# ingonyama-zk/blaze

Measured on AMD Instinct MI355X. Metric: BLS12-381 MSM/s at 2^26, higher is better.
Workload: dtype u32 registers holding 28-bit limbs (381-bit Fq, Montgomery)

## Files before the change

### blaze_amd/csrc/arena.hip

```cpp
#include "msm_engine.hpp"

#include <atomic>
#include <cstdlib>
#include <string>

namespace blz {

static std::mutex g_arena_mu;
static std::map<int, Arena*> g_arenas;

Arena& arena_for(int device_id) {
    std::lock_guard<std::mutex> lk(g_arena_mu);
    auto it = g_arenas.find(device_id);
    if (it == g_arenas.end()) it = g_arenas.emplace(device_id, new Arena()).first;
    return *it->second;
}

ArenaExtent* arena_find(Arena& a, uint64_t pos, size_t len) {
    if (pos + len < pos) return nullptr;
    for (auto& e : a.ext)
        if (pos >= e.start && pos + len <= e.start + e.len) return &e;
    return nullptr;
}

uint32_t* arena_flag_acquire(Arena& a) {
    if (!a.build_flags) {
        if (hipMalloc((void**)&a.build_flags, 256 * sizeof(uint32_t)) != hipSuccess) {
            (void)hipGetLastError();
            a.build_flags = nullptr;
            return nullptr;
        }
        a.flag_free.clear();
        for (int i = 255; i >= 0; --i) a.flag_free.push_back((uint16_t)i);
    }
    if (a.flag_free.empty()) return nullptr;
    uint32_t* f = a.build_flags + a.flag_free.back();
    a.flag_free.pop_back();
    return f;
}
void arena_flag_release(Arena& a, uint32_t*& f) {
    if (f && a.build_flags && f >= a.build_flags && f < a.build_flags + 256) a.flag_free.push_back((uint16_t)(f - a.build_flags));
    f = nullptr;
}

void arena_drop_build(Arena& a, ArenaExtent& x) {
    if (x.build.tab) (void)hipFree(x.build.tab);
    if (x.build.done) (void)hipEventDestroy(x.build.done);
    if (x.build.t0) (void)hipEventDestroy(x.build.t0);
    arena_flag_release(a, x.build.flag);
    x.build = ArenaExtent::TableBuild();
}
void arena_drop_table(Arena& a, ArenaExtent& x) {
    for (auto& t : x.tables)
        if (t.p) (void)hipFree(t.p);
    x.tables.clear();
    x.tab_dirty_lo = x.tab_dirty_hi = 0;
    arena_drop_build(a, x);
}

void arena_free_extent(Arena& a, ArenaExtent& x) {
    if (x.raw) {
        if (x.imported) (void)hipIpcCloseMemHandle(x.raw);
        else (void)hipFree(x.raw);
    }
    if (x.mont) (void)hipFree(x.mont);
    arena_drop_table(a, x);
    if (x.shadow_ready) (void)hipEventDestroy(x.shadow_ready);
    if (x.diet_ev) (void)hipEventDestroy(x.diet_ev);
    arena_flag_release(a, x.diet_flag);
    x = ArenaExtent();
}

uint64_t arena_next_epoch() {
    static std::atomic<uint64_t> next{1};
    return next.fetch_add(1);
}

static size_t format_point_bytes(int format_id) { return (format_id & 0xff) == BLZ_BN254 ? 64 : 96; }

int arena_restore_raw(Arena& a, ArenaExtent& e, hipStream_t st) {
    (void)a;
    if (e.diet == 1) e.diet = 0;
    if (e.diet != 2) return BLZ_OK;
    const size_t ps = format_point_bytes(e.mont_curve), mp = mont_point_bytes(e.mont_curve & 0xff);
    void* raw = nullptr;
    BLZ_HIP(hipMalloc(&raw, e.cap), BLZ_ERR_UNKNOWN);
    int rc = msm_points_from_mont(e.mont_curve, e.mont, raw, e.len / ps, st);
    if (rc == BLZ_OK) rc = sync_stream_bounded(st, "arena: raw bytes back from the Montgomery copy");
    if (rc != BLZ_OK) {
        if (!wait_timed_out()) (void)hipFree(raw);
// ... 280 lines not shown
```

### blaze_amd/csrc/arena_tables.hip

```cpp
#include <chrono>
#include <thread>

#include "msm_handle.hpp"

namespace blz {

bool wants_table_mode(const blz_msm* h) { return h->pf == 1 && h->window_table != 0; }

int arena_points_mont(blz_msm* h, uint64_t pos, uint32_t npts, const void** out, bool even) {
    *out = nullptr;
    const size_t ps = point_size(h), mp = mont_point_bytes(h->curve);
    const size_t len = (size_t)npts * ps;
    Arena& A = arena_for(h->device);
    std::lock_guard<std::mutex> lk(A.mu);
    ArenaExtent* e = arena_find(A, pos, len);
    if (!e)
        return fail(BLZ_ERR_INVALID_PARAM, "HBM bases: no loaded extent covers [%llu, +%zu) on device %d",
                    (unsigned long long)pos, len, h->device);
    const uint32_t phase = (uint32_t)((pos - e->start) % ps);
    const size_t cap_pts = (e->cap - phase) / ps, ext_pts = (e->len - phase) / ps;
    const uint64_t first = (pos - e->start - phase) / ps;
    if (even) {
        const ArenaExtent::PrecompCheck& C = e->pcheck;
        if ((first & 7u) || C.state != 1 || C.curve != h->curve || C.phase != phase || first < C.first || first + npts > C.first + C.npts) return BLZ_OK;
    }
    const int fmt = h->eng.format_id() | (even ? 1 << 16 : 0);
    const size_t want_bytes = (even ? (cap_pts / 8) * 4 : cap_pts) * mp;
    if (e->mont_curve != fmt || e->mont_phase != phase || e->mont_bytes < want_bytes) {
        BLZ_TRY(arena_restore_raw(A, *e, h->eng.stream));
        if (e->mont) {
            BLZ_TRY(sync_device_bounded("replacing a Montgomery shadow"));
            (void)hipFree(e->mont);
            e->mont = nullptr;
        }
        e->mont_bytes = want_bytes + 16;
        BLZ_HIP(hipMalloc(&e->mont, e->mont_bytes), BLZ_ERR_UNKNOWN);
        e->mont_curve = fmt;
        e->mont_phase = phase;
        e->dirty_lo = 0;
        e->dirty_hi = e->len;
        e->shadow_recorded = false;
    }
    if (!e->shadow_ready) BLZ_HIP(hipEventCreateWithFlags(&e->shadow_ready, hipEventDisableTiming), BLZ_ERR_UNKNOWN);
    if (e->shadow_recorded) BLZ_HIP(hipStreamWaitEvent(h->eng.stream, e->shadow_ready, 0), BLZ_ERR_UNKNOWN);
    if (e->dirty_lo < e->dirty_hi) {
        uint64_t lo = e->dirty_lo > phase ? (e->dirty_lo - phase) / ps : 0;
        uint64_t hi = e->dirty_hi > phase ? (e->dirty_hi - phase + ps - 1) / ps : 0;
        if (hi > ext_pts) hi = ext_pts;
        if (even) {
            const uint64_t elo = lo / 8, ehi = hi / 8 < ext_pts / 8 ? (hi + 7) / 8 : ext_pts / 8;
            if (elo < ehi)
                BLZ_TRY(h->eng.points_to_mont_even((const char*)e->raw + phase + elo * 8 * ps, (char*)e->mont + elo * 4 * mp, (uint32_t)((ehi - elo) * 4)));
        } else if (lo < hi) {
            BLZ_TRY(h->eng.points_to_mont((const char*)e->raw + phase + lo * ps, (char*)e->mont + lo * mp, (uint32_t)(hi - lo)));
        }
        BLZ_HIP(hipEventRecord(e->shadow_ready, h->eng.stream), BLZ_ERR_UNKNOWN);
        e->shadow_recorded = true;
        e->dirty_lo = e->dirty_hi = 0;
    }
    *out = (const char*)e->mont + (even ? first / 8 * 4 : first) * mp;
    if (even) h->pc_info[3] = e->mont_bytes;
    else if (!wants_table_mode(h)) BLZ_TRY(arena_diet_step(A, *e, ps, h->eng.stream));
    return BLZ_OK;
}

int arena_precompute_check(blz_msm* h, uint64_t pos, uint32_t nelem, bool* ok, uint64_t* checked_elems) {
    *ok = false;
    if (checked_elems) *checked_elems = nelem;
    const size_t ps = point_size(h);
// ... 76 lines not shown
    std::lock_guard<std::mutex> lk(A.mu);
    if (kernel_done) arena_flag_release(A, flag);
    BLZ_TRY(rc);
    ArenaExtent* e = arena_find(A, pos, len);
    if (!e || e->epoch != epoch) {
        BLZ_LOG(1, "precompute plan: the extent was written while its table was being checked: exact path for this task");
        return BLZ_OK;
    }
    ArenaExtent::PrecompCheck& C = e->pcheck;
    if (C.gen != gen) {
        BLZ_LOG(1, "precompute plan: another check of the extent committed while this one ran: exact path for this task");
        return BLZ_OK;
    }
    ++C.gen;
    C.state = flag_h ? 2 : 1;
    C.curve = h->curve;
    C.phase = phase;
    if (!partial) {
        C.first = first;
        C.npts = (uint64_t)nelem * 8;
    }
    C.redo_lo = C.redo_hi = 0;
    C.ms = ms;
    *ok = flag_h == 0;
    if (checked_elems) *checked_elems = C.npts / 8;
    h->pc_info[1] = (uint64_t)C.state;
    h->pc_info[2] = (uint64_t)(ms * 1000.0f);
    BLZ_LOG(1, "precompute plan: %s%llu elements checked: the table %s (%.1f ms)", partial ? "rewritten span, " : "", (unsigned long long)chk_elems,
            flag_h ? "is NOT B_j = 2^32 B_(j-1) over on-curve bases: exact path (8n points, 32-bit chunks)" : "is consistent: 4n even bases, 64-bit chunks", ms);
    return BLZ_OK;
}

constexpr uint32_t TABLE_BUILD_CHUNK = 3u << 16;
int arena_points_table(blz_msm* h, uint64_t pos, uint32_t npts, const void** out, int* c_out, int chunk_budget) {
    *out = nullptr;
    *c_out = 0;
    const size_t ps = point_size(h), mp = mont_point_bytes(h->curve);
    const size_t len = (size_t)npts * ps;
    Arena& A = arena_for(h->device);
    std::lock_guard<std::mutex> lk(A.mu);
    ArenaExtent* e = arena_find(A, pos, len);
    if (!e)
        return fail(BLZ_ERR_INVALID_PARAM, "HBM bases: no loaded extent covers [%llu, +%zu) on device %d",
                    (unsigned long long)pos, len, h->device);
    if (npts == 0) return BLZ_OK;
    BLZ_TRY(arena_restore_raw(A, *e, h->eng.stream));
    const uint32_t phase = (uint32_t)((pos - e->start) % ps);
    const uint64_t first = (pos - e->start - phase) / ps;
    const int fmt = h->eng.format_id();
    const int lo = h->range_hi ? h->range_lo : 0, hi = h->range_hi ? h->range_hi : 256;
    const int need = hi - lo < 256 ? hi - lo + 1 : 257;
    const int want_c = table_window_bits(npts, need);
    if (want_c == 0) return BLZ_OK;
    ArenaExtent::TableBuild& B = e->build;
    auto enqueue_chunks = [&](int budget) -> int {
        hipStream_t st = h->eng.stream;
        const uint64_t nchunks = (B.npts + TABLE_BUILD_CHUNK - 1) / TABLE_BUILD_CHUNK;
        if (B.next_chunk >= nchunks || budget == 0) return BLZ_OK;
        if (!A.scratch_event) BLZ_HIP(hipEventCreateWithFlags(&A.scratch_event, hipEventDisableTiming), BLZ_ERR_UNKNOWN);
        if (A.scratch_recorded) BLZ_HIP(hipStreamWaitEvent(st, A.scratch_event, 0), BLZ_ERR_UNKNOWN);
        for (; B.next_chunk < nchunks && budget != 0; ++B.next_chunk, --budget) {
            const uint64_t p0 = B.next_chunk * TABLE_BUILD_CHUNK;
            const uint32_t cnt = (uint32_t)(B.npts - p0 < TABLE_BUILD_CHUNK ? B.npts - p0 : TABLE_BUILD_CHUNK);
            if (B.next_chunk == 0) BLZ_HIP(hipEventRecord(B.t0, st), BLZ_ERR_UNKNOWN);
            BLZ_TRY(h->eng.build_table((const char*)e->raw + B.phase + (B.first + p0) * ps, (char*)B.tab + p0 * (size_t)B.W * mp, cnt, B.c, B.W, B.lo,
                                       A.build_scratch, B.flag, st));
        }
        BLZ_HIP(hipEventRecord(B.done, st), BLZ_ERR_UNKNOWN);
        B.recorded = true;
        BLZ_HIP(hipEventRecord(A.scratch_event, st), BLZ_ERR_UNKNOWN);
        A.scratch_recorded = true;
        return BLZ_OK;
    };
    hipError_t bq = hipErrorNotReady;
    if (B.tab) {
        const uint64_t nchunks = (B.npts + TABLE_BUILD_CHUNK - 1) / TABLE_BUILD_CHUNK;
        if (B.next_chunk >= nchunks && B.recorded) {
            bq = hipEventQuery(B.done);
            if (bq != hipSuccess && bq != hipErrorNotReady) { (void)hipGetLastError(); return fail(BLZ_ERR_UNKNOWN, "window table build failed: %s", hipGetErrorString(bq)); }
        }
    }
    if (B.tab && bq == hipSuccess) {
        uint32_t flag_h = 0;
        float ms = 0;
        BLZ_HIP(hipMemcpy(&flag_h, B.flag, 4, hipMemcpyDeviceToHost), BLZ_ERR_READ);
        (void)hipEventElapsedTime(&ms, B.t0, B.done);
        if (flag_h) {
            BLZ_LOG(1, "window table: a base has a multiple at infinity (a point of even order): plain path for this extent");
            BLZ_TRY(sync_device_bounded("dropping a refused window table"));
            (void)hipFree(B.tab);
            (void)hipEventDestroy(B.done);
            (void)hipEventDestroy(B.t0);
            arena_flag_release(A, B.flag);
            B = ArenaExtent::TableBuild();
            e->table_refused = true;
            return BLZ_OK;
        }
        ArenaExtent::WindowTable t;
        t.p = B.tab;
        t.bytes = B.bytes;
        t.format = B.format;
        t.phase = B.phase;
        t.first = B.first;
        t.npts = B.npts;
        t.c = B.c;
        t.W = B.W;
        t.lo = B.lo;
        t.hi = B.hi;
        t.build_ms = ms;
        e->tables.push_back(t);
        B.tab = nullptr;
        (void)hipEventDestroy(B.done);
        (void)hipEventDestroy(B.t0);
        arena_flag_release(A, B.flag);
        B = ArenaExtent::TableBuild();
        BLZ_LOG(1, "window table: %llu bases x %d windows of %d bits, %.1f MiB, complete %.1f ms after its first chunk", (unsigned long long)t.npts,
                t.W, t.c, t.bytes / 1048576.0, ms);
    }
    if (e->tab_dirty_lo < e->tab_dirty_hi && !e->tables.empty()) {
        BLZ_TRY(sync_device_bounded("window table: drain before the rewritten bases are re-tabulated"));
        uint32_t* pflag = arena_flag_acquire(A);
        if (pflag && hipMemsetAsync(pflag, 0, 4, h->eng.stream) != hipSuccess) {
            (void)hipGetLastError();
            arena_flag_release(A, pflag);
        }
        bool patched = false;
        for (size_t k = e->tables.size(); k-- > 0;) {
            ArenaExtent::WindowTable& t = e->tables[k];
            const uint64_t plo = e->tab_dirty_lo > t.phase ? (e->tab_dirty_lo - t.phase) / ps : 0;
            const uint64_t phi = e->tab_dirty_hi > t.phase ? (e->tab_dirty_hi - t.phase + ps - 1) / ps : 0;
            const uint64_t lo_p = plo > t.first ? plo : t.first, hi_p = phi < t.first + t.npts ? phi : t.first + t.npts;
            if (lo_p >= hi_p) continue;
            if (t.format != fmt || !pflag || A.build_scratch_bytes < h->eng.table_scratch_bytes(t.W) + 16) {
                (void)hipFree(t.p);
                e->tables.erase(e->tables.begin() + (long)k);
                continue;
            }
            BLZ_TRY(h->eng.build_table((const char*)e->raw + t.phase + lo_p * ps, (char*)t.p + (lo_p - t.first) * (size_t)t.W * mp, (uint32_t)(hi_p - lo_p), t.c,
                                       t.W, t.lo, A.build_scratch, pflag, h->eng.stream));
            patched = true;
        }
        if (!patched) arena_flag_release(A, pflag);
        if (patched) {
            uint32_t flag_h = 0;
            BLZ_WAIT(h, sync_stream_bounded(h->eng.stream, "window table: rewritten bases re-tabulated"));
            const hipError_t he_flag = hipMemcpy(&flag_h, pflag, 4, hipMemcpyDeviceToHost);
            arena_flag_release(A, pflag);
            BLZ_HIP(he_flag, BLZ_ERR_READ);
            if (flag_h) {
                BLZ_LOG(1, "window table: a rewritten base has a multiple at infinity (a point of even order): plain path for this extent");
                arena_drop_table(A, *e);
                e->table_refused = true;
                return BLZ_OK;
            }
            BLZ_LOG(1, "window table: rows of the rewritten bases re-tabulated (bytes [%llu, %llu) of the extent)", (unsigned long long)e->tab_dirty_lo,
                    (unsigned long long)e->tab_dirty_hi);
        }
        e->tab_dirty_lo = e->tab_dirty_hi = 0;
    }
    const ArenaExtent::WindowTable* T = nullptr;
    for (const auto& t : e->tables)
        if (t.format == fmt && t.phase == phase && first >= t.first && first + npts <= t.first + t.npts && t.lo == lo && t.hi == hi) T = &t;
    if (T && T->c != want_c) return BLZ_OK;
    if (!T) {
        if (B.tab) {
            if (B.format == fmt && B.phase == phase && first >= B.first && first + npts <= B.first + B.npts && B.lo == lo && B.hi == hi)
                BLZ_TRY(enqueue_chunks(chunk_budget));
            return BLZ_OK;
        }
        if (e->table_refused) return BLZ_OK;
        if (e->tables.size() >= ArenaExtent::MAX_TABLES) {
            BLZ_LOG(1, "window table: the extent already holds %zu tables: plain path for this handle", e->tables.size());
            return BLZ_OK;
        }
        const int c = want_c, W = table_windows(c, need);
        const size_t bytes = (size_t)npts * W * mp + 16;
        size_t free_b = 0, total_b = 0;
        BLZ_HIP(hipMemGetInfo(&free_b, &total_b), BLZ_ERR_UNKNOWN);
        const size_t scratch_b = h->eng.table_scratch_bytes(W) + 16;
        const size_t workspace = (size_t)npts * W * 32 + ((size_t)1 << (c - 1)) * 256 + ((size_t)1 << 30);
        if (free_b < bytes + scratch_b + workspace) {
            BLZ_LOG(1, "window table: %zu bytes for %u bases (c = %d, %d windows) do not fit beside the workspace (%zu free): plain path",
                    bytes, npts, c, W, free_b);
            e->table_refused = true;
            return BLZ_OK;
        }
        if (A.build_scratch_bytes < scratch_b) {
            if (A.build_scratch) {
                BLZ_TRY(sync_device_bounded("growing the window-table scratch"));
                (void)hipFree(A.build_scratch);
                A.build_scratch = nullptr;
                A.build_scratch_bytes = 0;
            }
            if (hipMalloc(&A.build_scratch, scratch_b) != hipSuccess) {
                (void)hipGetLastError();
                A.build_scratch = nullptr;
                e->table_refused = true;
                return BLZ_OK;
            }
            A.build_scratch_bytes = scratch_b;
        }
        void* tab = nullptr;
        const auto t_alloc = std::chrono::steady_clock::now();
        const hipError_t he_tab = hipMalloc(&tab, bytes);
        BLZ_LOG(1, "window table: hipMalloc(%zu) took %.1f ms", bytes,
                std::chrono::duration<double, std::milli>(std::chrono::steady_clock::now() - t_alloc).count());
        if (he_tab != hipSuccess) {
            (void)hipGetLastError();
            e->table_refused = true;
            return BLZ_OK;
        }
        hipEvent_t done = nullptr, t0 = nullptr;
        int rc = BLZ_OK;
        if (hipEventCreate(&t0) != hipSuccess || hipEventCreate(&done) != hipSuccess) rc = fail_hip(BLZ_ERR_UNKNOWN, "event creation failed");
        uint32_t* flag = arena_flag_acquire(A);
        if (!flag) {
            (void)hipFree(tab);
            if (t0) (void)hipEventDestroy(t0);
            if (done) (void)hipEventDestroy(done);
            e->table_refused = true;
            return BLZ_OK;
        }
        if (rc == BLZ_OK && hipMemsetAsync(flag, 0, 4, h->eng.stream) != hipSuccess) rc = fail_hip(BLZ_ERR_UNKNOWN, "memset failed");
        if (rc != BLZ_OK) {
            if (t0) (void)hipEventDestroy(t0);
            if (done) (void)hipEventDestroy(done);
            (void)hipFree(tab);
            arena_flag_release(A, flag);
            return rc;
        }
        B.tab = tab;
        B.flag = flag;
        B.bytes = bytes;
        B.done = done;
        B.t0 = t0;
        B.format = fmt;
        B.c = c;
        B.W = W;
        B.lo = lo;
        B.hi = hi;
        B.phase = phase;
        B.first = first;
        B.npts = npts;
        B.next_chunk = 0;
        B.recorded = false;
        BLZ_LOG(1, "window table: build of %u bases x %d windows of %d bits started (%.1f MiB, %u chunks); tasks take the plain path until it is there",
                npts, W, c, bytes / 1048576.0, (unsigned)((npts + TABLE_BUILD_CHUNK - 1) / TABLE_BUILD_CHUNK));
        return enqueue_chunks(chunk_budget);
    }
    *out = (const char*)T->p + (first - T->first) * (size_t)T->W * mp;
    *c_out = T->c;
    h->table_info[0] = T->bytes;
    h->table_info[1] = (uint64_t)T->c;
    h->table_info[2] = (uint64_t)T->W;
    h->table_info[3] = (uint64_t)(T->build_ms * 1000.0f);
    return BLZ_OK;
}

bool wants_table(const blz_msm* h) {
    return h->pf == 1 && (h->window_table == 2 || (h->window_table == 1 && h->curve != BLZ_BN254));
}

int plan_repr_bn254(uint64_t nelem) {
    const int forced = plan_override("pc_repr", -1);
    if (forced == 0 || forced == 1) return forced;
    return nelem > (1ull << 25) ? 1 : 0;
}

void task_repr_bn254pc(blz_msm* h, bool on_plan, uint64_t checked_elems) {
    if (h->curve != BLZ_BN254 || h->pf != BLZ_PRECOMPUTE_FACTOR || busy(h)) return;
    h->eng.repr = exp_knob("BLAZE_BN254_REPR", on_plan ? plan_repr_bn254(checked_elems) : 1) ? 1 : 0;
}

int resolve_arena_task(blz_msm* h, uint64_t pos, uint32_t n, bool allow_table, bool allow_plan, uint32_t* npts, int* sbits, int* table_c,
                       const void** pts) {
    *npts = n * h->pf;
    *sbits = h->pf == 1 ? 256 : 32;
    *table_c = 0;
    memset(h->table_info, 0, sizeof(h->table_info));
    memset(h->pc_info, 0, sizeof(h->pc_info));
    if (h->pf == BLZ_PRECOMPUTE_FACTOR && h->precompute_plan && allow_plan && n > 0) {
        bool ok = false;
        uint64_t checked = n;
        BLZ_TRY(arena_precompute_check(h, pos, n, &ok, &checked));
        const bool plan = ok && h->eng.plan_for(n * 4, 64).c != 0;
        task_repr_bn254pc(h, plan, checked);
        if (plan) {
            const void* even = nullptr;
            BLZ_TRY(arena_points_mont(h, pos, n * 8, &even, true));
            if (even) {
                *pts = even;
                *npts = n * 4;
                *sbits = 64;
                h->pc_info[0] = 1;
                return BLZ_OK;
            }
            h->pc_info[1] = 0;
            task_repr_bn254pc(h, false, 0);
        }
    } else {
        task_repr_bn254pc(h, false, 0);
    }
    if (allow_table && wants_table(h)) {
        const void* tab = nullptr;
        BLZ_TRY(arena_points_table(h, pos, *npts, &tab, table_c, TABLE_CHUNKS_PER_TASK));
        if (tab) *pts = tab;
        else *table_c = 0;
    }
    if (!*table_c) BLZ_TRY(arena_points_mont(h, pos, *npts, pts));
    return BLZ_OK;
}

}
```

### blaze_amd/csrc/common.hip

```cpp
#include "common.hpp"

#include <condition_variable>
#include <memory>

#include <chrono>
#include <cstdlib>
#include <thread>

namespace blz {

static thread_local char g_err[1024] = "";

void set_last_error(const char* fmt, ...) {
    va_list ap;
    va_start(ap, fmt);
    vsnprintf(g_err, sizeof(g_err), fmt, ap);
    va_end(ap);
    BLZ_LOG(1, "error: %s", g_err);
}

int log_level() {
    static int lvl = -1;
    if (lvl < 0) {
        const char* s = getenv("BLAZE_LOG");
// ... 2 lines not shown
    return lvl;
}

int device_count() {
    int n = 0;
    hipError_t e = hipGetDeviceCount(&n);
    if (e != hipSuccess) {
        (void)hipGetLastError();
        return 0;
    }
    return n;
}

int use_device(int device_id) {
    int n = device_count();
    if (device_id < 0 || device_id >= n)
        return fail(BLZ_ERR_FILE, "no HIP device with ordinal %d (%d visible); this library has no CPU path", device_id, n);
    BLZ_HIP(hipSetDevice(device_id), BLZ_ERR_FILE);
    return BLZ_OK;
}

int env_int(const char* name, int dflt) {
    const char* s = getenv(name);
    return s && *s ? atoi(s) : dflt;
}

int plan_override(const char* key, int dflt) {
    const char* s = getenv("BLAZE_MSM_PLAN");
    if (!s || !*s) return dflt;
    const size_t kl = strlen(key);
    for (const char* p = s; *p;) {
        while (*p == ',' || *p == ' ') ++p;
        if (strncmp(p, key, kl) == 0 && p[kl] == '=') return atoi(p + kl + 1);
        while (*p && *p != ',') ++p;
    }
    return dflt;
}

int wait_timeout_ms() {
    const char* s = getenv("BLAZE_WAIT_TIMEOUT_MS");
    int v = s && *s ? atoi(s) : 120000;
    return v > 0 ? v : 120000;
}

static thread_local bool g_wait_timed_out = false;
bool wait_timed_out() { return g_wait_timed_out; }
void wait_clear() { g_wait_timed_out = false; }

template <class Q>
static int bounded_wait(Q&& query, const char* what) {
    g_wait_timed_out = false;
    const auto t0 = std::chrono::steady_clock::now();
    const int limit_ms = wait_timeout_ms();
    for (;;) {
        hipError_t e = query();
        if (e == hipSuccess) return BLZ_OK;
        if (e != hipErrorNotReady) {
            (void)hipGetLastError();
            return fail_hip(BLZ_ERR_UNKNOWN, "%s failed: %s", what, hipGetErrorString(e));
        }
        const auto dt = std::chrono::steady_clock::now() - t0;
        if (dt > std::chrono::milliseconds(limit_ms)) {
            g_wait_timed_out = true;
            return fail(BLZ_ERR_UNKNOWN, "%s timed out after %d ms (BLAZE_WAIT_TIMEOUT_MS): the device task did not complete; "
                        "the handle accepts only reset / free now", what, limit_ms);
        }
// ... 33 lines not shown
    const int limit_ms = wait_timeout_ms();
    if (!job->cv.wait_for(lk, std::chrono::milliseconds(limit_ms), [&] { return job->done; })) {
        g_wait_timed_out = true;
        return fail(BLZ_ERR_UNKNOWN, "%s timed out after %d ms (BLAZE_WAIT_TIMEOUT_MS): device work in flight did not complete; the "
                    "buffers it may still touch are leaked, not freed", what, limit_ms);
    }
    if (job->err != hipSuccess) {
        (void)hipGetLastError();
        return fail_hip(BLZ_ERR_UNKNOWN, "%s failed: %s", what, hipGetErrorString(job->err));
    }
    return BLZ_OK;
}

int DevBuf::reserve(size_t bytes, bool exact) {
    if (bytes <= cap) return BLZ_OK;
    if (p) {
        const int rc = sync_device_bounded("growing a device buffer");
        if (rc != BLZ_OK) {
            p = nullptr;
            cap = 0;
            return rc;
        }
        (void)hipFree(p);
        p = nullptr;
        cap = 0;
    }
    size_t want = exact ? bytes : bytes + bytes / 8;
    hipError_t e = hipMalloc(&p, want);
    if (e != hipSuccess) {
        e = hipMalloc(&p, bytes);
        want = bytes;
    }
    if (e != hipSuccess) {
        p = nullptr;
        return fail_hip(BLZ_ERR_UNKNOWN, "hipMalloc(%zu) failed: %s", bytes, hipGetErrorString(e));
    }
    cap = want;
    return BLZ_OK;
}

int ensure_dynamic_lds(const void* kernel, int bytes) {
    static std::mutex mu;
    static std::map<std::pair<int, const void*>, int> done;
    int dev = 0;
    BLZ_HIP(hipGetDevice(&dev), BLZ_ERR_UNKNOWN);
    std::lock_guard<std::mutex> lk(mu);
    auto key = std::make_pair(dev, kernel);
    auto it = done.find(key);
    if (it != done.end() && it->second >= bytes) return BLZ_OK;
    BLZ_HIP(hipFuncSetAttribute(kernel, hipFuncAttributeMaxDynamicSharedMemorySize, bytes), BLZ_ERR_UNKNOWN);
    done[key] = bytes;
    return BLZ_OK;
}

}

extern "C" {

const char* blz_last_error_message(void) { return blz::g_err; }
int blz_device_count(void) { return blz::device_count(); }
size_t blz_point_size(int curve) { return curve == BLZ_BN254 ? 64 : (curve == BLZ_BLS377 || curve == BLZ_BLS381) ? 96 : 0; }
size_t blz_result_size(int curve) { return curve == BLZ_BN254 ? 96 : (curve == BLZ_BLS377 || curve == BLZ_BLS381) ? 144 : 0; }

int blz_device_malloc(int device_id, size_t bytes, void** out) {
    if (!out) return blz::fail(BLZ_ERR_INVALID_PARAM, "null out");
    BLZ_TRY(blz::use_device(device_id));
// ... 33 lines not shown
```

### blaze_amd/csrc/common.hpp

```cpp
#pragma once
#include <hip/hip_runtime.h>
#include <cstdarg>
#include <cstdint>
#include <cstdio>
#include <cstring>
#include <map>
#include <mutex>
#include <string>
#include <vector>

#include "../../include/blaze_hip.h"
#include "../../include/blaze_hip_aux.h"

namespace blz {

void set_last_error(const char* fmt, ...);
int log_level();

#define BLZ_LOG(lvl, ...)                                  \
    do {                                                   \
        if (::blz::log_level() >= (lvl)) {                 \
            fprintf(stderr, "[blaze_hip] " __VA_ARGS__);   \
            fputc('\n', stderr);                           \
        }                                                  \
// ... 13 lines not shown
#define BLZ_TRY(expr)              \
    do {                           \
        int rc__ = (expr);         \
        if (rc__ != BLZ_OK) return rc__; \
    } while (0)

inline int fail(int code, const char* fmt, ...) {
    char buf[512];
    va_list ap;
    va_start(ap, fmt);
    vsnprintf(buf, sizeof(buf), fmt, ap);
    va_end(ap);
    set_last_error("%s", buf);
    return code;
}
inline int fail_hip(int code, const char* fmt, ...) {
    char buf[512];
    va_list ap;
    va_start(ap, fmt);
    vsnprintf(buf, sizeof(buf), fmt, ap);
    va_end(ap);
    set_last_error("%s", buf);
    (void)hipGetLastError();
    return code;
}

int env_int(const char* name, int dflt);
#ifdef BLZ_EXPERIMENT_KNOBS
inline int exp_knob(const char* name, int dflt) { return env_int(name, dflt); }
#else
inline int exp_knob(const char*, int dflt) { return dflt; }
#endif
int plan_override(const char* key, int dflt);

int device_count();
int use_device(int device_id);

int wait_timeout_ms();
int sync_event_bounded(hipEvent_t ev, const char* what);
int sync_stream_bounded(hipStream_t st, const char* what);
int sync_device_bounded(const char* what);
bool wait_timed_out();
void wait_clear();

int ensure_dynamic_lds(const void* kernel, int bytes);

struct DevBuf {
    void* p = nullptr;
    size_t cap = 0;
    int reserve(size_t bytes, bool exact = false);
    void release() {
        if (p) (void)hipFree(p);
        p = nullptr;
        cap = 0;
    }
    template <class T>
    T* as() const { return reinterpret_cast<T*>(p); }
};

struct ArenaExtent {
    uint64_t start = 0;
    size_t len = 0, cap = 0;
    void* raw = nullptr;
    bool imported = false;
    bool exported = false;
    void* mont = nullptr;
    size_t mont_bytes = 0;
    int mont_curve = -1;
    uint32_t mont_phase = 0;
    uint64_t dirty_lo = 0, dirty_hi = 0;
    hipEvent_t shadow_ready = nullptr;
    bool shadow_recorded = false;
    struct WindowTable {
        void* p = nullptr;
        size_t bytes = 0;
        int format = -1, c = 0, W = 0;
        int lo = 0, hi = 256;
        uint32_t phase = 0;
        uint64_t first = 0, npts = 0;
        float build_ms = 0;
    };
    static constexpr size_t MAX_TABLES = 32;
    static constexpr uint64_t TABLE_PATCH_MAX_POINTS = 1u << 18;
    std::vector<WindowTable> tables;
    uint64_t tab_dirty_lo = 0, tab_dirty_hi = 0;
    bool table_refused = false;
    struct PrecompCheck {
        int state = 0;
        int curve = -1;
        uint32_t phase = 0;
        uint64_t first = 0, npts = 0;
        uint64_t redo_lo = 0, redo_hi = 0;
        float ms = 0;
        uint64_t gen = 0;
    } pcheck;
    int diet = 0;
    hipEvent_t diet_ev = nullptr;
    uint32_t* diet_flag = nullptr;
    uint64_t epoch = 0;
    struct TableBuild {
        void* tab = nullptr;
        uint32_t* flag = nullptr;
        size_t bytes = 0;
        hipEvent_t done = nullptr, t0 = nullptr;
        int format = -1, c = 0, W = 0, lo = 0, hi = 256;
        uint32_t phase = 0;
        uint64_t first = 0, npts = 0;
        uint64_t next_chunk = 0;
        bool recorded = false;
    } build;
};
struct Arena {
    std::mutex mu;
    std::vector<ArenaExtent> ext;
    void* build_scratch = nullptr;
    size_t build_scratch_bytes = 0;
    hipEvent_t scratch_event = nullptr;
    bool scratch_recorded = false;
    uint32_t* build_flags = nullptr;
    std::vector<uint16_t> flag_free;
    int policy = 0;
};
Arena& arena_for(int device_id);
ArenaExtent* arena_find(Arena& a, uint64_t pos, size_t len);
int arena_write(int device_id, uint64_t pos, const void* src, size_t len, bool src_is_device, hipStream_t st);
void arena_free_extent(Arena& a, ArenaExtent& x);
uint32_t* arena_flag_acquire(Arena& a);
void arena_flag_release(Arena& a, uint32_t*& f);
uint64_t arena_next_epoch();
int arena_restore_raw(Arena& a, ArenaExtent& e, hipStream_t st);
int arena_diet_step(Arena& a, ArenaExtent& e, size_t point_bytes, hipStream_t st);
int arena_read_bytes(Arena& a, ArenaExtent& e, uint64_t off, size_t len, void* out, hipStream_t st);
void arena_drop_table(Arena& a, ArenaExtent& x);
void arena_drop_build(Arena& a, ArenaExtent& x);

}
```

### blaze_amd/csrc/msm_capi.hip

```cpp
#include <chrono>
#include <thread>

#include "msm_handle.hpp"

using namespace blz;

extern "C" {

int blz_msm_new(int device_id, int mem_type, int is_precompute, int curve, blz_msm** out) {
    if (!out) return fail(BLZ_ERR_INVALID_PARAM, "null out");
    *out = nullptr;
    if (curve < 0 || curve > 2) return fail(BLZ_ERR_INVALID_PARAM, "unknown curve %d", curve);
    if (mem_type != BLZ_HBM && mem_type != BLZ_DMA) return fail(BLZ_ERR_INVALID_PARAM, "unknown mem_type %d", mem_type);
    BLZ_TRY(use_device(device_id));
    blz_msm* h = new blz_msm();
    h->device = device_id;
    h->mem_type = mem_type;
    h->pf = is_precompute ? BLZ_PRECOMPUTE_FACTOR : BLZ_PRECOMPUTE_FACTOR_BASE;
    h->curve = curve;
    h->window_table = 0;
    int rc = h->eng.init(device_id, curve, (int)h->pf);
    if (rc == BLZ_OK && hipStreamCreateWithFlags(&h->copy_stream, hipStreamNonBlocking) != hipSuccess)
        rc = fail_hip(BLZ_ERR_UNKNOWN, "copy stream creation failed");
    for (int i = 0; i < 2 && rc == BLZ_OK; ++i)
        if (hipEventCreateWithFlags(&h->set_free[i], hipEventDisableTiming) != hipSuccess)
            rc = fail_hip(BLZ_ERR_UNKNOWN, "event creation failed");
    for (int i = 0; i < blz_msm::PieceRing::SLOTS && rc == BLZ_OK; ++i)
        if (hipEventCreateWithFlags(&h->ring.raw_read[i], hipEventDisableTiming) != hipSuccess)
            rc = fail_hip(BLZ_ERR_UNKNOWN, "event creation failed");
    if (rc != BLZ_OK) {
        h->eng.destroy();
        delete h;
        return rc;
    }
    *out = h;
    return BLZ_OK;
}

void blz_msm_free(blz_msm* h) {
    if (!h) return;
    (void)hipSetDevice(h->device);
    if (h->comm) (void)blz_msm_comm_free(h);
    if (!h->eng.destroy() || sync_stream_bounded(h->copy_stream, "free: copy stream") != BLZ_OK) {
        delete h;
        return;
    }
    if (h->copy_stream) (void)hipStreamDestroy(h->copy_stream);
    for (int i = 0; i < 2; ++i) {
        h->scalars_buf[i].release();
        h->points_raw[i].release();
        if (h->set_free[i]) (void)hipEventDestroy(h->set_free[i]);
    }
    h->points_mont.release();
// ... 351 lines not shown
```

### blaze_amd/csrc/msm_handle.hpp

```cpp
#pragma once
#include <deque>

#include "msm_engine.hpp"
#include "rccl_dyn.hpp"

struct blz_msm {
    int device = 0;
    int mem_type = BLZ_DMA;
    uint32_t pf = 1;
    int curve = BLZ_BLS381;
    uint32_t nof_elements = 0;
    bool bases_from_hbm = false;
    uint64_t hbm_addr = 0;
    bool initialized = false;
    struct Pending { int slot; uint32_t label; };
    std::deque<Pending> in_flight;
    uint32_t task_label = 0;
    struct Res { std::vector<uint8_t> bytes; uint32_t label; };
    std::deque<Res> results;
    blz::DevBuf scalars_buf[2], points_raw[2], points_mont;
    hipEvent_t set_free[2] = {nullptr, nullptr};
    bool set_used[2] = {false, false};
    int stage_idx = 0;
    hipStream_t copy_stream = nullptr;
    struct PieceRing {
        static constexpr int SLOTS = 4;
        blz::DevBuf raw, mont;
        uint64_t slot_pts = 0;
        hipEvent_t raw_read[SLOTS] = {nullptr, nullptr, nullptr, nullptr};
        bool recorded[SLOTS] = {false, false, false, false};
        uint64_t next = 0;
    } ring;
    struct Feed {
        bool armed = false;
        bool open = false;
        bool ready = false;
        int mode = 0;
        bool src_device = false;
        uint32_t n = 0;
        uint32_t received = 0;
        int set = -1;
        const void* d_scalars = nullptr;
        uint64_t arena_pos = 0;
        int slot = -1;
        uint32_t per = 0;
        uint32_t ppe = 1;
        uint32_t npts = 0;
        int sbits = 0;
        bool even = false;
        uint64_t ring_first = 0;
        const void* mont = nullptr;
    } feed;
    blz::MsmEngine eng;
    bool wedged = false;
    ncclComm_t comm = nullptr;
    int comm_rank = 0, comm_size = 0;
    blz::DevBuf comm_buf;
    int window_table = 0;
    int range_lo = 0, range_hi = 0;
    uint64_t table_info[4] = {0, 0, 0, 0};
    int precompute_plan = 0;
    uint64_t pc_info[4] = {0, 0, 0, 0};
};

namespace blz {

#define BLZ_LIVE(h)                                                                                              \
    do {                                                                                                         \
        if ((h)->wedged)                                                                                         \
            return fail(BLZ_ERR_UNKNOWN, "handle is wedged: an earlier wait timed out (BLAZE_WAIT_TIMEOUT_MS); only " \
                                         "reset / free are accepted");                                           \
    } while (0)
#define BLZ_WAIT(h, expr)                          \
    do {                                           \
        wait_clear();                              \
        int rc__ = (expr);                         \
        if (rc__ != BLZ_OK) {                      \
            if (wait_timed_out()) (h)->wedged = true; \
            return rc__;                           \
        }                                          \
    } while (0)

#define BLZ_ARENA_ADDR(addr, off)                                                                                          \
    do {                                                                                                                   \
        if ((uint64_t)(addr) + (uint64_t)(off) < (uint64_t)(addr))                                                         \
            return fail(BLZ_ERR_INVALID_PARAM, "HBM address %llu + offset %llu wraps around 2^64", (unsigned long long)(addr), \
                        (unsigned long long)(off));                                                                        \
    } while (0)

inline size_t point_size(const blz_msm* h) { return blz_point_size(h->curve); }
inline size_t result_size(const blz_msm* h) { return blz_result_size(h->curve); }
inline bool busy(const blz_msm* h) { return !h->in_flight.empty() || h->feed.slot >= 0; }

constexpr int TABLE_CHUNKS_PER_TASK = 4;
bool wants_table_mode(const blz_msm* h);
bool wants_table(const blz_msm* h);
int plan_repr_bn254(uint64_t nelem);
void task_repr_bn254pc(blz_msm* h, bool on_plan, uint64_t checked_elems);
int arena_points_mont(blz_msm* h, uint64_t pos, uint32_t npts, const void** out, bool even = false);
int arena_precompute_check(blz_msm* h, uint64_t pos, uint32_t nelem, bool* ok, uint64_t* checked_elems = nullptr);
int arena_points_table(blz_msm* h, uint64_t pos, uint32_t npts, const void** out, int* c_out, int chunk_budget);
int resolve_arena_task(blz_msm* h, uint64_t pos, uint32_t n, bool allow_table, bool allow_plan, uint32_t* npts, int* sbits, int* table_c,
                       const void** pts);
int launch_if_ready(blz_msm* h);
int stage(blz_msm* h, const void* points, size_t points_len, const void* scalars, size_t scalars_len, uint32_t m, int has_hbm,
          uint64_t hbm_addr, uint64_t hbm_off, bool on_device);
void feed_abandon(blz_msm* h);

}
```

### blaze_amd/csrc/msm_stage.hip

```cpp
#include "msm_handle.hpp"

namespace blz {

static int task_enqueued(blz_msm* h, int slot) {
    if (h->feed.set >= 0) h->set_used[h->feed.set] = true;
    h->in_flight.push_back({slot, h->task_label});
    h->feed = blz_msm::Feed();
    return BLZ_OK;
}

void feed_abandon(blz_msm* h) {
    blz_msm::Feed& F = h->feed;
    if (F.slot >= 0) h->eng.abandon(F.slot);
    if (F.set >= 0) h->set_used[F.set] = true;
    const bool armed = F.armed;
    F = blz_msm::Feed();
    F.armed = armed;
}

int launch_if_ready(blz_msm* h) {
    const blz_msm::Feed& F = h->feed;
    if (!(F.armed && F.ready)) return BLZ_OK;
    if (!h->eng.can_accept())
        return fail(BLZ_ERR_INVALID_PARAM, "task queue full (%d in flight); call wait_result first", MSM_QUEUE_DEPTH);
    uint32_t npts = F.n * h->pf;
    int sbits = h->pf == 1 ? 256 : 32;
    int slot = 0;
    int table_c = 0;
    const void* pts = h->points_mont.p;
    memset(h->table_info, 0, sizeof(h->table_info));
    memset(h->pc_info, 0, sizeof(h->pc_info));
    if (F.mode != 2) BLZ_TRY(resolve_arena_task(h, F.arena_pos, F.n, true, F.mode == 1, &npts, &sbits, &table_c, &pts));
    h->eng.inputs_event = F.set >= 0 ? h->set_free[F.set] : nullptr;
    BLZ_TRY(h->eng.run(pts, F.d_scalars, npts, sbits, &slot, table_c, h->range_lo, h->range_hi));
    return task_enqueued(h, slot);
}

static int pick_pieces(const blz_msm* h, uint32_t npts, bool with_points) {
    int pieces = env_int("BLAZE_MSM_PIECES", 0);
    if (pieces <= 0) {
        if (with_points) {
            pieces = (int)(npts >> 19);
            if (npts >= (1u << 20) && npts <= (1u << 21)) pieces = (int)(npts >> 18);
            if (pieces > 16) pieces = 16;
            if (busy(h) && pieces > 4) pieces = 4;
        } else {
            pieces = (int)(npts >> 23);
            if (pieces > 8) pieces = 8;
            if (pieces < 4) pieces = 4;
        }
    }
    return pieces < 1 ? 1 : pieces;
}

static int ring_reserve(blz_msm* h, uint32_t piece_pts) {
    blz_msm::PieceRing& R = h->ring;
    if (piece_pts <= R.slot_pts) return BLZ_OK;
    R.slot_pts = 0;
    for (bool& r : R.recorded) r = false;
    const size_t ps = point_size(h), mp = mont_point_bytes(h->curve);
    BLZ_TRY(R.raw.reserve((size_t)piece_pts * blz_msm::PieceRing::SLOTS * ps + 16, true));
    BLZ_TRY(R.mont.reserve((size_t)piece_pts * blz_msm::PieceRing::SLOTS * mp + 16, true));
    R.slot_pts = piece_pts;
    return BLZ_OK;
}

static int ring_slot(blz_msm* h, uint64_t k, char** raw, char** mont) {
// ... 41 lines not shown
        const uint64_t want = F.arena_pos + (uint64_t)F.received * h->pf * ps;
        if (mode == 3 && pos != want)
            return fail(BLZ_ERR_INVALID_PARAM, "slice of a streamed task: its points go to %llu, behind the %u elements already loaded at %llu (got %llu)",
                        (unsigned long long)want, F.received, (unsigned long long)F.arena_pos, (unsigned long long)pos);
        return BLZ_OK;
    }
    if ((uint64_t)n * h->pf >= (1ull << 31)) return fail(BLZ_ERR_INVALID_PARAM, "too many points");
    if (n && h->eng.plan_for(n * h->pf, h->pf == 1 ? 256 : 32).c == 0)
        return fail(BLZ_ERR_INVALID_PARAM, "no window plan for %llu points of %d-bit scalars (u32 entry indexing: at most 352321536 points at pf = 1, 2113929216 at pf = 8)",
                    (unsigned long long)n * h->pf, h->pf == 1 ? 256 : 32);
    if (!h->eng.can_accept())
        return fail(BLZ_ERR_INVALID_PARAM, "task queue full (%d in flight); call wait_result first", MSM_QUEUE_DEPTH);
    if (on_device && m == n) {
        if (((uintptr_t)scalars) % 16) return fail(BLZ_ERR_INVALID_PARAM, "device scalars must be 16-byte aligned");
        if (mode == 2 && ((uintptr_t)points) % 16) return fail(BLZ_ERR_INVALID_PARAM, "device points must be 16-byte aligned");
    }
    if (mode == 1) {
        Arena& A = arena_for(h->device);
        std::lock_guard<std::mutex> lk(A.mu);
        if (!arena_find(A, pos, (size_t)n * h->pf * ps))
            return fail(BLZ_ERR_INVALID_PARAM, "HBM bases: no loaded extent covers [%llu, +%zu) on device %d", (unsigned long long)pos,
                        (size_t)n * h->pf * ps, h->device);
    }
    return BLZ_OK;
}

static int open_pieces(blz_msm* h, bool one_call) {
    blz_msm::Feed& F = h->feed;
    if (!F.armed || F.n == 0 || F.set < 0 || (F.mode == 3 && !one_call) || exp_knob("BLAZE_DMA_OVERLAP", 1) == 0) return BLZ_OK;
    uint32_t npts = F.n * h->pf;
    int sbits = h->pf == 1 ? 256 : 32;
    const void* mont = nullptr;
    if (F.mode != 2) {
        if (!(npts >= (1u << 22) || env_int("BLAZE_MSM_PIECES", 0) > 1) || busy(h) || wants_table(h)) return BLZ_OK;
        int tc = 0;
        BLZ_TRY(resolve_arena_task(h, F.arena_pos, F.n, false, F.mode == 1, &npts, &sbits, &tc, &mont));
    }
    const int want = pick_pieces(h, npts, F.mode == 2);
    if (!one_call && want < 2) return BLZ_OK;
    int slot = -1;
    h->eng.inputs_event = h->set_free[F.set];
    BLZ_TRY(h->eng.begin(npts, sbits, &slot, 0, h->range_lo, h->range_hi, want, true));
    const int pieces = h->eng.slots[slot].slices;
    if (!one_call && pieces < 2) {
        h->eng.abandon(slot);
        return BLZ_OK;
    }
    F.slot = slot;
    F.per = h->eng.slots[slot].pts_per_slice;
    F.npts = npts;
    F.sbits = sbits;
    F.ppe = npts / F.n;
    F.even = h->pc_info[0] != 0;
    F.mont = mont;
    if (F.mode == 2) {
        BLZ_TRY(ring_reserve(h, F.per));
        F.ring_first = h->ring.next;
        h->ring.next += (uint64_t)pieces;
    }
    return BLZ_OK;
}

static int open_feed(blz_msm* h, int mode, bool on_device, const void* scalars, uint32_t n, uint32_t m, uint64_t pos) {
    feed_abandon(h);
    blz_msm::Feed& F = h->feed;
    F.open = true;
    F.mode = mode;
// ... 141 lines not shown
```

Before: 8.134.

## Auto-build window tables for HBM bases reused across tasks, release under memory pressure

Handles now default to an automatic window-table policy: when the same large HBM base extent is used by a second task, a precomputed window table is built in full and later MSMs use the table path instead of the plain Montgomery path. Reuse is tracked per extent by task label and epoch, and pieces-based DMA overlap is skipped when an auto table applies. To avoid out-of-memory failures, auto-built tables are capped at a memory budget and freed on allocation failure, with a retry. The risk is that the first repeat task pays the full table-build cost synchronously, and the extra device memory can push other allocations into eviction.

Measured after the change: 9.147 (median of 6 runs). 1.12x the previous value.

```diff
diff --git a/blaze_amd/csrc/arena.hip b/blaze_amd/csrc/arena.hip
--- a/blaze_amd/csrc/arena.hip
+++ b/blaze_amd/csrc/arena.hip
@@ -56,6 +56,65 @@
     x.tables.clear();
     x.tab_dirty_lo = x.tab_dirty_hi = 0;
     arena_drop_build(a, x);
+}
+
+static thread_local const void* g_table_pin = nullptr;
+static thread_local bool g_table_pin_skipped = false;
+void table_pin(const void* rows) {
+    g_table_pin = rows;
+    g_table_pin_skipped = false;
+}
+bool table_pin_skipped() { return g_table_pin_skipped; }
+
+size_t arena_release_auto_tables(Arena& a) {
+    auto pinned = [](const ArenaExtent::WindowTable& t) {
+        return g_table_pin && (const char*)g_table_pin >= (const char*)t.p && (const char*)g_table_pin < (const char*)t.p + t.bytes;
+    };
+    bool any = false;
+    for (const auto& x : a.ext) {
+        if (x.build.tab && x.build.auto_built) any = true;
+        for (const auto& t : x.tables) {
+            if (!t.auto_built) continue;
+            if (pinned(t)) g_table_pin_skipped = true;
+            else any = true;
+        }
+    }
+    if (!any) return 0;
+    if (sync_device_bounded("memory pressure: drain before the auto-built window tables go") != BLZ_OK) return 0;
+    size_t freed = 0;
+    for (auto& x : a.ext) {
+        bool dropped = false;
+        if (x.build.tab && x.build.auto_built) {
+            freed += x.build.bytes;
+            arena_drop_build(a, x);
+            dropped = true;
+        }
+        for (size_t k = x.tables.size(); k-- > 0;) {
+            if (!x.tables[k].auto_built || pinned(x.tables[k])) continue;
+            freed += x.tables[k].bytes;
+            (void)hipFree(x.tables[k].p);
+            x.tables.erase(x.tables.begin() + (long)k);
+            dropped = true;
+        }
+        if (!dropped) continue;
+        if (x.tables.empty()) x.tab_dirty_lo = x.tab_dirty_hi = 0;
+        x.table_refused = true;
+        x.reuse = ArenaExtent::Reuse();
+    }
+    (void)hipGetLastError();
+    BLZ_LOG(1, "window table: memory pressure - %zu bytes of auto-built tables released; their extents take the plain path until the next write", freed);
+    return freed;
+}
+
+size_t release_auto_tables_on_oom() {
+    int dev = 0;
+    if (hipGetDevice(&dev) != hipSuccess) {
+        (void)hipGetLastError();
+        return 0;
+    }
+    Arena& A = arena_for(dev);
+    std::lock_guard<std::mutex> lk(A.mu);
+    return arena_release_auto_tables(A);
 }
 
 void arena_free_extent(Arena& a, ArenaExtent& x) {
diff --git a/blaze_amd/csrc/arena_tables.hip b/blaze_amd/csrc/arena_tables.hip
--- a/blaze_amd/csrc/arena_tables.hip
+++ b/blaze_amd/csrc/arena_tables.hip
@@ -5,7 +5,11 @@
 
 namespace blz {
 
-bool wants_table_mode(const blz_msm* h) { return h->pf == 1 && h->window_table != 0; }
+bool wants_table_mode(const blz_msm* h) { return h->pf == 1 && h->window_table > 0; }
+
+bool auto_table_handle(const blz_msm* h) {
+    return h->window_table < 0 && h->pf == 1 && h->mem_type == BLZ_HBM && h->curve != BLZ_BN254 && plan_override("auto_table", 1) != 0;
+}
 
 int arena_points_mont(blz_msm* h, uint64_t pos, uint32_t npts, const void** out, bool even) {
     *out = nullptr;
@@ -34,7 +38,18 @@
             e->mont = nullptr;
         }
         e->mont_bytes = want_bytes + 16;
-        BLZ_HIP(hipMalloc(&e->mont, e->mont_bytes), BLZ_ERR_UNKNOWN);
+        hipError_t he_mont = hipMalloc(&e->mont, e->mont_bytes);
+        if (he_mont != hipSuccess) {
+            (void)hipGetLastError();
+            e->mont = nullptr;
+            if (arena_release_auto_tables(A) > 0) he_mont = hipMalloc(&e->mont, e->mont_bytes);
+        }
+        if (he_mont != hipSuccess) {
+            e->mont = nullptr;
+            e->mont_bytes = 0;
+            e->mont_curve = -1;
+            return fail_hip(BLZ_ERR_UNKNOWN, "hipMalloc of a Montgomery copy failed: %s", hipGetErrorString(he_mont));
+        }
         e->mont_curve = fmt;
         e->mont_phase = phase;
         e->dirty_lo = 0;
@@ -177,7 +192,7 @@
 }
 
 constexpr uint32_t TABLE_BUILD_CHUNK = 3u << 16;
-int arena_points_table(blz_msm* h, uint64_t pos, uint32_t npts, const void** out, int* c_out, int chunk_budget) {
+int arena_points_table(blz_msm* h, uint64_t pos, uint32_t npts, const void** out, int* c_out, int chunk_budget, bool auto_policy) {
     *out = nullptr;
     *c_out = 0;
     const size_t ps = point_size(h), mp = mont_point_bytes(h->curve);
@@ -189,7 +204,7 @@
         return fail(BLZ_ERR_INVALID_PARAM, "HBM bases: no loaded extent covers [%llu, +%zu) on device %d",
                     (unsigned long long)pos, len, h->device);
     if (npts == 0) return BLZ_OK;
-    BLZ_TRY(arena_restore_raw(A, *e, h->eng.stream));
+    if (!auto_policy) BLZ_TRY(arena_restore_raw(A, *e, h->eng.stream));
     const uint32_t phase = (uint32_t)((pos - e->start) % ps);
     const uint64_t first = (pos - e->start - phase) / ps;
     const int fmt = h->eng.format_id();
@@ -198,6 +213,25 @@
     const int want_c = table_window_bits(npts, need);
     if (want_c == 0) return BLZ_OK;
     ArenaExtent::TableBuild& B = e->build;
+    if (auto_policy) {
+        ArenaExtent::Reuse& R = e->reuse;
+        const bool same_task = R.count && R.last_handle == h && R.last_label == h->task_label;
+        R.last_handle = h;
+        R.last_label = h->task_label;
+        if (same_task && R.format == fmt && R.phase == phase && R.first == first && R.npts == npts && R.lo == lo && R.hi == hi && R.epoch == e->epoch) {
+        } else if (R.count && R.format == fmt && R.phase == phase && R.first == first && R.npts == npts && R.lo == lo && R.hi == hi && R.epoch == e->epoch) {
+            if (R.count < 0xffffffffu) ++R.count;
+        } else {
+            R.format = fmt;
+            R.phase = phase;
+            R.first = first;
+            R.npts = npts;
+            R.lo = lo;
+            R.hi = hi;
+            R.epoch = e->epoch;
+            R.count = 1;
+        }
+    }
     auto enqueue_chunks = [&](int budget) -> int {
         hipStream_t st = h->eng.stream;
         const uint64_t nchunks = (B.npts + TABLE_BUILD_CHUNK - 1) / TABLE_BUILD_CHUNK;
@@ -253,6 +287,7 @@
         t.lo = B.lo;
         t.hi = B.hi;
         t.build_ms = ms;
+        t.auto_built = B.auto_built;
         e->tables.push_back(t);
         B.tab = nullptr;
         (void)hipEventDestroy(B.done);
@@ -262,7 +297,13 @@
         BLZ_LOG(1, "window table: %llu bases x %d windows of %d bits, %.1f MiB, complete %.1f ms after its first chunk", (unsigned long long)t.npts,
                 t.W, t.c, t.bytes / 1048576.0, ms);
     }
-    if (e->tab_dirty_lo < e->tab_dirty_hi && !e->tables.empty()) {
+    bool patch_rows = e->tab_dirty_lo < e->tab_dirty_hi && !e->tables.empty();
+    if (patch_rows && auto_policy) {
+        patch_rows = false;
+        for (const auto& t : e->tables) patch_rows = patch_rows || t.auto_built;
+        if (patch_rows) BLZ_TRY(arena_restore_raw(A, *e, h->eng.stream));
+    }
+    if (patch_rows) {
         BLZ_TRY(sync_device_bounded("window table: drain before the rewritten bases are re-tabulated"));
         uint32_t* pflag = arena_flag_acquire(A);
         if (pflag && hipMemsetAsync(pflag, 0, 4, h->eng.stream) != hipSuccess) {
@@ -306,14 +347,17 @@
     const ArenaExtent::WindowTable* T = nullptr;
     for (const auto& t : e->tables)
         if (t.format == fmt && t.phase == phase && first >= t.first && first + npts <= t.first + t.npts && t.lo == lo && t.hi == hi) T = &t;
+    if (T && auto_policy && !T->auto_built) return BLZ_OK;
     if (T && T->c != want_c) return BLZ_OK;
     if (!T) {
         if (B.tab) {
-            if (B.format == fmt && B.phase == phase && first >= B.first && first + npts <= B.first + B.npts && B.lo == lo && B.hi == hi)
-                BLZ_TRY(enqueue_chunks(chunk_budget));
+            if (B.format == fmt && B.phase == phase && first >= B.first && first + npts <= B.first + B.npts && B.lo == lo && B.hi == hi &&
+                (!auto_policy || B.auto_built))
+                BLZ_TRY(enqueue_chunks(B.auto_built ? -1 : chunk_budget));
             return BLZ_OK;
         }
         if (e->table_refused) return BLZ_OK;
+        if (auto_policy && (npts < (uint32_t)plan_override("auto_table_min", 1 << 24) || e->reuse.count < 2)) return BLZ_OK;
         if (e->tables.size() >= ArenaExtent::MAX_TABLES) {
             BLZ_LOG(1, "window table: the extent already holds %zu tables: plain path for this handle", e->tables.size());
             return BLZ_OK;
@@ -329,6 +373,17 @@
                     bytes, npts, c, W, free_b);
             e->table_refused = true;
             return BLZ_OK;
+        }
+        if (auto_policy) {
+            const long long cap_env = plan_override_ll("table_budget_bytes", -1);
+            const size_t cap = cap_env >= 0 ? (size_t)cap_env : free_b / 2;
+            if (bytes > cap) {
+                BLZ_LOG(1, "window table: auto policy: %zu bytes for %u bases exceed the budget (%zu: %s): plain path until the next write", bytes,
+                        npts, cap, cap_env >= 0 ? "table_budget_bytes" : "half of the free device memory");
+                e->table_refused = true;
+                return BLZ_OK;
+            }
+            BLZ_TRY(arena_restore_raw(A, *e, h->eng.stream));
         }
         if (A.build_scratch_bytes < scratch_b) {
             if (A.build_scratch) {
@@ -389,9 +444,11 @@
         B.npts = npts;
         B.next_chunk = 0;
         B.recorded = false;
-        BLZ_LOG(1, "window table: build of %u bases x %d windows of %d bits started (%.1f MiB, %u chunks); tasks take the plain path until it is there",
-                npts, W, c, bytes / 1048576.0, (unsigned)((npts + TABLE_BUILD_CHUNK - 1) / TABLE_BUILD_CHUNK));
-        return enqueue_chunks(chunk_budget);
+        B.auto_built = auto_policy;
+        BLZ_LOG(1, "window table: %sbuild of %u bases x %d windows of %d bits started (%.1f MiB, %u chunks); tasks take the plain path until it is there",
+                auto_policy ? "auto policy (second task over the same bases): " : "", npts, W, c, bytes / 1048576.0,
+                (unsigned)((npts + TABLE_BUILD_CHUNK - 1) / TABLE_BUILD_CHUNK));
+        return enqueue_chunks(auto_policy ? -1 : chunk_budget);
     }
     *out = (const char*)T->p + (first - T->first) * (size_t)T->W * mp;
     *c_out = T->c;
@@ -404,6 +461,27 @@
 
 bool wants_table(const blz_msm* h) {
     return h->pf == 1 && (h->window_table == 2 || (h->window_table == 1 && h->curve != BLZ_BN254));
+}
+
+bool wants_table_for(const blz_msm* h, uint64_t pos, uint32_t npts) {
+    if (wants_table(h)) return true;
+    if (!auto_table_handle(h)) return false;
+    Arena& A = arena_for(h->device);
+    std::lock_guard<std::mutex> lk(A.mu);
+    const size_t ps = point_size(h);
+    const ArenaExtent* e = arena_find(A, pos, (size_t)npts * ps);
+    if (!e) return false;
+    const uint32_t phase = (uint32_t)((pos - e->start) % ps);
+    const uint64_t first = (pos - e->start - phase) / ps;
+    const int fmt = h->eng.format_id();
+    const int lo = h->range_hi ? h->range_lo : 0, hi = h->range_hi ? h->range_hi : 256;
+    const ArenaExtent::TableBuild& B = e->build;
+    if (B.tab && B.auto_built && B.format == fmt && B.phase == phase && first >= B.first && first + npts <= B.first + B.npts && B.lo == lo && B.hi == hi)
+        return true;
+    for (const auto& t : e->tables)
+        if (t.auto_built && t.format == fmt && t.phase == phase && first >= t.first && first + npts <= t.first + t.npts && t.lo == lo && t.hi == hi)
+            return true;
+    return false;
 }
 
 int plan_repr_bn254(uint64_t nelem) {
@@ -446,11 +524,13 @@
     } else {
         task_repr_bn254pc(h, false, 0);
     }
-    if (allow_table && wants_table(h)) {
+    const bool auto_policy = allow_plan && auto_table_handle(h);
+    if ((allow_table && wants_table(h)) || auto_policy) {
         const void* tab = nullptr;
-        BLZ_TRY(arena_points_table(h, pos, *npts, &tab, table_c, TABLE_CHUNKS_PER_TASK));
-        if (tab) *pts = tab;
+        BLZ_TRY(arena_points_table(h, pos, *npts, &tab, table_c, TABLE_CHUNKS_PER_TASK, auto_policy));
+        if (tab && allow_table) *pts = tab;
         else *table_c = 0;
+        if (!*table_c) memset(h->table_info, 0, sizeof(h->table_info));
     }
     if (!*table_c) BLZ_TRY(arena_points_mont(h, pos, *npts, pts));
     return BLZ_OK;
diff --git a/blaze_amd/csrc/common.hip b/blaze_amd/csrc/common.hip
--- a/blaze_amd/csrc/common.hip
+++ b/blaze_amd/csrc/common.hip
@@ -58,6 +58,18 @@
     for (const char* p = s; *p;) {
         while (*p == ',' || *p == ' ') ++p;
         if (strncmp(p, key, kl) == 0 && p[kl] == '=') return atoi(p + kl + 1);
+        while (*p && *p != ',') ++p;
+    }
+    return dflt;
+}
+
+long long plan_override_ll(const char* key, long long dflt) {
+    const char* s = getenv("BLAZE_MSM_PLAN");
+    if (!s || !*s) return dflt;
+    const size_t kl = strlen(key);
+    for (const char* p = s; *p;) {
+        while (*p == ',' || *p == ' ') ++p;
+        if (strncmp(p, key, kl) == 0 && p[kl] == '=') return atoll(p + kl + 1);
         while (*p && *p != ',') ++p;
     }
     return dflt;
@@ -157,6 +169,10 @@
         want = bytes;
     }
     if (e != hipSuccess) {
+        (void)hipGetLastError();
+        if (release_auto_tables_on_oom() > 0) e = hipMalloc(&p, bytes);
+    }
+    if (e != hipSuccess) {
         p = nullptr;
         return fail_hip(BLZ_ERR_UNKNOWN, "hipMalloc(%zu) failed: %s", bytes, hipGetErrorString(e));
     }
diff --git a/blaze_amd/csrc/common.hpp b/blaze_amd/csrc/common.hpp
--- a/blaze_amd/csrc/common.hpp
+++ b/blaze_amd/csrc/common.hpp
@@ -69,6 +69,7 @@
 inline int exp_knob(const char*, int dflt) { return dflt; }
 #endif
 int plan_override(const char* key, int dflt);
+long long plan_override_ll(const char* key, long long dflt);
 
 int device_count();
 int use_device(int device_id);
@@ -116,6 +117,7 @@
         uint32_t phase = 0;
         uint64_t first = 0, npts = 0;
         float build_ms = 0;
+        bool auto_built = false;
     };
     static constexpr size_t MAX_TABLES = 32;
     static constexpr uint64_t TABLE_PATCH_MAX_POINTS = 1u << 18;
@@ -145,7 +147,16 @@
         uint64_t first = 0, npts = 0;
         uint64_t next_chunk = 0;
         bool recorded = false;
+        bool auto_built = false;
     } build;
+    struct Reuse {
+        int format = -1, lo = 0, hi = 256;
+        uint32_t phase = 0;
+        uint64_t first = 0, npts = 0, epoch = 0;
+        uint32_t count = 0;
+        const void* last_handle = nullptr;
+        uint32_t last_label = 0;
+    } reuse;
 };
 struct Arena {
     std::mutex mu;
@@ -170,5 +181,9 @@
 int arena_read_bytes(Arena& a, ArenaExtent& e, uint64_t off, size_t len, void* out, hipStream_t st);
 void arena_drop_table(Arena& a, ArenaExtent& x);
 void arena_drop_build(Arena& a, ArenaExtent& x);
+size_t arena_release_auto_tables(Arena& a);
+size_t release_auto_tables_on_oom();
+void table_pin(const void* table_rows);
+bool table_pin_skipped();
 
 }
diff --git a/blaze_amd/csrc/msm_capi.hip b/blaze_amd/csrc/msm_capi.hip
--- a/blaze_amd/csrc/msm_capi.hip
+++ b/blaze_amd/csrc/msm_capi.hip
@@ -18,7 +18,7 @@
     h->mem_type = mem_type;
     h->pf = is_precompute ? BLZ_PRECOMPUTE_FACTOR : BLZ_PRECOMPUTE_FACTOR_BASE;
     h->curve = curve;
-    h->window_table = 0;
+    h->window_table = -1;
     int rc = h->eng.init(device_id, curve, (int)h->pf);
     if (rc == BLZ_OK && hipStreamCreateWithFlags(&h->copy_stream, hipStreamNonBlocking) != hipSuccess)
         rc = fail_hip(BLZ_ERR_UNKNOWN, "copy stream creation failed");
diff --git a/blaze_amd/csrc/msm_handle.hpp b/blaze_amd/csrc/msm_handle.hpp
--- a/blaze_amd/csrc/msm_handle.hpp
+++ b/blaze_amd/csrc/msm_handle.hpp
@@ -56,7 +56,7 @@
     ncclComm_t comm = nullptr;
     int comm_rank = 0, comm_size = 0;
     blz::DevBuf comm_buf;
-    int window_table = 0;
+    int window_table = -1;
     int range_lo = 0, range_hi = 0;
     uint64_t table_info[4] = {0, 0, 0, 0};
     int precompute_plan = 0;
@@ -95,11 +95,13 @@
 constexpr int TABLE_CHUNKS_PER_TASK = 4;
 bool wants_table_mode(const blz_msm* h);
 bool wants_table(const blz_msm* h);
+bool auto_table_handle(const blz_msm* h);
+bool wants_table_for(const blz_msm* h, uint64_t pos, uint32_t npts);
 int plan_repr_bn254(uint64_t nelem);
 void task_repr_bn254pc(blz_msm* h, bool on_plan, uint64_t checked_elems);
 int arena_points_mont(blz_msm* h, uint64_t pos, uint32_t npts, const void** out, bool even = false);
 int arena_precompute_check(blz_msm* h, uint64_t pos, uint32_t nelem, bool* ok, uint64_t* checked_elems = nullptr);
-int arena_points_table(blz_msm* h, uint64_t pos, uint32_t npts, const void** out, int* c_out, int chunk_budget);
+int arena_points_table(blz_msm* h, uint64_t pos, uint32_t npts, const void** out, int* c_out, int chunk_budget, bool auto_policy = false);
 int resolve_arena_task(blz_msm* h, uint64_t pos, uint32_t n, bool allow_table, bool allow_plan, uint32_t* npts, int* sbits, int* table_c,
                        const void** pts);
 int launch_if_ready(blz_msm* h);
diff --git a/blaze_amd/csrc/msm_stage.hip b/blaze_amd/csrc/msm_stage.hip
--- a/blaze_amd/csrc/msm_stage.hip
+++ b/blaze_amd/csrc/msm_stage.hip
@@ -30,9 +30,16 @@
     const void* pts = h->points_mont.p;
     memset(h->table_info, 0, sizeof(h->table_info));
     memset(h->pc_info, 0, sizeof(h->pc_info));
-    if (F.mode != 2) BLZ_TRY(resolve_arena_task(h, F.arena_pos, F.n, true, F.mode == 1, &npts, &sbits, &table_c, &pts));
-    h->eng.inputs_event = F.set >= 0 ? h->set_free[F.set] : nullptr;
-    BLZ_TRY(h->eng.run(pts, F.d_scalars, npts, sbits, &slot, table_c, h->range_lo, h->range_hi));
+    for (int attempt = 0;; ++attempt) {
+        if (F.mode != 2) BLZ_TRY(resolve_arena_task(h, F.arena_pos, F.n, true, F.mode == 1, &npts, &sbits, &table_c, &pts));
+        h->eng.inputs_event = F.set >= 0 ? h->set_free[F.set] : nullptr;
+        table_pin(table_c ? pts : nullptr);
+        const int rc = h->eng.run(pts, F.d_scalars, npts, sbits, &slot, table_c, h->range_lo, h->range_hi);
+        const bool skipped = table_pin_skipped();
+        table_pin(nullptr);
+        if (rc == BLZ_OK) break;
+        if (!(attempt == 0 && skipped && !wait_timed_out() && release_auto_tables_on_oom() > 0)) return rc;
+    }
     return task_enqueued(h, slot);
 }
 
@@ -140,7 +147,7 @@
     int sbits = h->pf == 1 ? 256 : 32;
     const void* mont = nullptr;
     if (F.mode != 2) {
-        if (!(npts >= (1u << 22) || env_int("BLAZE_MSM_PIECES", 0) > 1) || busy(h) || wants_table(h)) return BLZ_OK;
+        if (!(npts >= (1u << 22) || env_int("BLAZE_MSM_PIECES", 0) > 1) || busy(h) || wants_table_for(h, F.arena_pos, npts)) return BLZ_OK;
         int tc = 0;
         BLZ_TRY(resolve_arena_task(h, F.arena_pos, F.n, false, F.mode == 1, &npts, &sbits, &tc, &mont));
     }
```
